# ziatdinovmax/GPim

Hardware: AMD Instinct MI355X
Metric: GP fit+predict grid-points/sec (higher is better)
Workload: dtype f64; 1 GPU; C2: 256x256 synthetic twisted-lattice image, 25% observed (N=16384, M=65536, d=2), Matern52 exact GP, T=100 Adam its (lr 0.1) + predict; one image per GPU; N=16384, M=65536, kernel=Matern52

## Files before the change

### gpim_amd/_lib.py

```python
import contextlib
import ctypes
import os

import torch

_HERE = os.path.dirname(os.path.abspath(__file__))
LIB_PATH = os.path.join(_HERE, "libgpimhip.so")

OK, E_BADARG, E_HIP, E_NOT_PD, E_NOMEM = 0, -1, -2, -3, -4
KERNEL_IDS = {"RBF": 0, "Matern52": 1, "RationalQuadratic": 2}
ACQ_IDS = {"cb": 0, "ei": 1, "poi": 2}
MAX_DIM, MAX_PARAMS = 4, 8

c_dp = ctypes.c_void_p


class ModelStruct(ctypes.Structure):
    _fields_ = [("kernel", ctypes.c_int32), ("dim", ctypes.c_int32), ("n_ls", ctypes.c_int32),
                ("reserved", ctypes.c_int32), ("amp_lo", ctypes.c_double), ("amp_hi", ctypes.c_double),
                ("ls_lo", ctypes.c_double * MAX_DIM), ("ls_hi", ctypes.c_double * MAX_DIM),
                ("jitter", ctypes.c_double)]


class VgpStruct(ctypes.Structure):
# ... 109 lines not shown
    "gpimhip_nll_grad_batched": (ctypes.c_int, [ctypes.c_void_p, ctypes.POINTER(ModelStruct), c_dp, ctypes.c_int64, c_dp,
                                                ctypes.c_int64, ctypes.c_int32, c_dp, c_dp, c_dp]),
    "gpimhip_acquire_exact": (ctypes.c_int, [ctypes.c_void_p, ctypes.POINTER(ModelStruct), c_dp, c_dp, ctypes.c_int64,
                                             c_dp, c_dp, ctypes.c_int64, c_dp, ctypes.c_int64, ctypes.c_int32,
                                             ctypes.c_double, ctypes.c_double, c_dp, c_dp, c_dp, c_dp]),
    "gpimhip_thin_batch": (ctypes.c_int, [ctypes.c_void_p, c_dp, c_dp, ctypes.c_int32, ctypes.c_int32, c_dp,
                                          ctypes.c_double, ctypes.c_int32, c_dp, c_dp]),
    "gpimhip_dist_vec_forward": (ctypes.c_int, [ctypes.c_void_p, c_dp, ctypes.c_int64, ctypes.c_int32, ctypes.c_int32,
                                                c_dp, c_dp, c_dp, c_dp]),
    "gpimhip_dist_vec_backward": (ctypes.c_int, [ctypes.c_void_p, c_dp, ctypes.c_int64, ctypes.c_int32, ctypes.c_int32,
                                                 c_dp, c_dp, c_dp, c_dp]),
    "gpimhip_matvec_t": (ctypes.c_int, [ctypes.c_void_p, c_dp, ctypes.c_int64, ctypes.c_int64, ctypes.c_int64, c_dp,
                                        c_dp]),
    "gpimhip_step_plan_host": (ctypes.c_int, [ctypes.c_int32, ctypes.c_int32, ctypes.POINTER(ctypes.c_int32),
                                              ctypes.c_int64, ctypes.POINTER(ctypes.c_int64)]),
    "gpimhip_step_plan_host_f32": (ctypes.c_int, [ctypes.c_int32, ctypes.c_int32, ctypes.POINTER(ctypes.c_int32),
                                                  ctypes.c_int64, ctypes.POINTER(ctypes.c_int64),
                                                  ctypes.POINTER(ctypes.c_int32)]),
    "gpimhip_vgp_nll_grad": (ctypes.c_int, [ctypes.c_void_p, ctypes.POINTER(ModelStruct), ctypes.POINTER(VgpStruct), c_dp,
                                            c_dp, ctypes.c_int64, c_dp, c_dp, c_dp]),
    "gpimhip_fit_vgp": (ctypes.c_int, [ctypes.c_void_p, ctypes.POINTER(ModelStruct), ctypes.POINTER(VgpStruct), c_dp, c_dp,
                                       ctypes.c_int64, c_dp, ctypes.c_double, ctypes.c_int32, c_dp, c_dp]),
    "gpimhip_predict_vgp": (ctypes.c_int, [ctypes.c_void_p, ctypes.POINTER(ModelStruct), ctypes.POINTER(VgpStruct), c_dp,
                                           c_dp, ctypes.c_int64, c_dp, c_dp, ctypes.c_int64, c_dp, c_dp]),
    "gpimhip_sm_kmat": (ctypes.c_int, [ctypes.c_void_p, ctypes.POINTER(SmStruct), c_dp, ctypes.c_int64, c_dp, ctypes.c_int64,
                                       c_dp, c_dp, ctypes.c_int64]),
    "gpimhip_sm_nll_grad": (ctypes.c_int, [ctypes.c_void_p, ctypes.POINTER(SmStruct), c_dp, c_dp, ctypes.c_int64, c_dp, c_dp,
                                           c_dp]),
    "gpimhip_fit_sm": (ctypes.c_int, [ctypes.c_void_p, ctypes.POINTER(SmStruct), c_dp, c_dp, ctypes.c_int64, c_dp,
                                      ctypes.c_double, ctypes.c_int32, c_dp, c_dp]),
# ... 124 lines not shown
```

### gpim_amd/csrc/api.hip

```cpp
#include <math.h>
#include <stdio.h>
#include <string.h>
#include <stdlib.h>
#include <algorithm>
#include <chrono>
#include <atomic>
#include <mutex>
#include "common.hpp"
#include "border.hpp"
#include "vgp.hpp"
#include "sm.hpp"
#include "sample.hpp"

static thread_local std::string g_err;
void gpim_set_error(const std::string& s) { g_err = s; }

static int deal_chunk(int ntiles = 1 << 30) { return std::max(1, std::min(64, ntiles / 512)); }
#define EAGER_MIN_PANELS 12
#define OUTER_W 4

template <typename T>
static int dev_alloc(gpimhip_ctx* h, T** p, int64_t count) {
    void* q = nullptr;
    hipError_t e = hipMalloc(&q, (size_t)count * sizeof(T));
    if (e != hipSuccess) {
        gpim_set_error(std::string("hipMalloc failed: ") + hipGetErrorString(e));
        return GPIMHIP_E_NOMEM;
    }
    *p = (T*)q;
    h->bytes += count * (int64_t)sizeof(T);
    return GPIMHIP_OK;
}
template <typename T>
static void dev_free(gpimhip_ctx* h, T** p, int64_t count) {
// ... 67 lines not shown
    }
    HIP_TRY(hipMemsetAsync(h->fin_counter, 0, (size_t)B * sizeof(uint32_t), h->stream));
    if (matrices) {
        HIP_TRY(hipMemsetAsync(h->Tm, 0, (size_t)mat_doubles(h, B * np * ld) * sizeof(double), h->stream));
        HIP_TRY(hipMemsetAsync(h->B, 0, (size_t)mat_doubles(h, B * np * ld) * sizeof(double), h->stream));
    }
    if (h->fp32 && h->refine_cap < 10 * (int64_t)B * np) {
        dev_free(h, &h->refine, h->refine_cap);
        h->refine_cap = 0;
        if ((rc = dev_alloc(h, &h->refine, 10 * (int64_t)B * np))) {
            ws_release_matrix(h);
            return rc;
        }
        h->refine_cap = 10 * (int64_t)B * np;
    }
    if (matrices) {
        rc = plan_ensure(h, (int)nb);
        if (rc == GPIMHIP_OK) rc = h->fp32 ? step_plan_ensure(h, (int)nb) : step_plan_ensure_inv(h, (int)nb);
        if (rc != GPIMHIP_OK) { ws_release_matrix(h); return rc; }
    }
    return GPIMHIP_OK;
}
int ws_ensure(gpimhip_ctx* h, int64_t N) { return ws_ensure_b(h, N, h->nbatch, 0); }
static int ws_ensure_padded(gpimhip_ctx* h, int64_t N) { return ws_ensure_b(h, N, h->nbatch, 1); }

static void ws_release_predict(gpimhip_ctx* h) {
    dev_free(h, &h->Ks, mat_doubles(h, h->ks_batch * h->ks_rows * (h->ks_cols + 16)));
    dev_free(h, &h->colpart, h->ks_batch * (h->ks_rows / NB) * h->ks_cols);
    dev_free(h, &h->mean_tmp, h->ks_batch * h->ks_cols);
    for (auto& pl : h->pred_lists) dev_free(h, &pl.tiles, pl.n);
// ... 127 lines not shown
    HIP_TRY(hipStreamSynchronize(h->stream));
    P.nb = nb;
    return GPIMHIP_OK;
}

static GemmArgs gemm_args(const double* A, int64_t lda, const double* B, int64_t ldb, double* C, int64_t ldc,
                          double alpha, double beta, const TileDesc* tiles, int n, int64_t rows) {
    GemmArgs g;
    memset(&g, 0, sizeof(g));
    g.A = A; g.lda = lda; g.B = B; g.ldb = ldb; g.C = C; g.ldc = ldc;
    g.alpha = alpha; g.beta = beta; g.tiles = tiles; g.ntiles = n;
    g.sA = rows * lda; g.sB = rows * ldb; g.sC = rows * ldc;
    return g;
}

struct SideStreams {
    hipStream_t capture = nullptr;
    bool capture_tried = false;
};
static std::mutex g_side_mutex;
static SideStreams g_side[64];
static std::atomic<int> g_side_generation{0};
static void side_refresh(gpimhip_ctx* h) {
    const int g = g_side_generation.load();
    if (h->side_generation == g) return;
    h->side_generation = g;
    h->capture_stream = nullptr;
    h->capture_stream_tried = false;
}
static std::mutex g_capture_mutex[64];
// ... 9 lines not shown
        if (!S.capture_tried) {
            S.capture_tried = true;
            if (hipStreamCreateWithFlags(&S.capture, hipStreamNonBlocking) != hipSuccess) S.capture = nullptr;
        }
        h->capture_stream = S.capture;
    }
    return h->capture_stream;
}

int launch_potrf(gpimhip_ctx* h, double* A, int64_t np, int64_t ld, int32_t* info) {
    return launch_potrf_steps(h, A, np, ld, info, nullptr);
}

int launch_trtri(gpimhip_ctx* h, double* A, double* Tm, int64_t np, int64_t ld) {
    const int nb = (int)(np / NB);
    GP_TRY(plan_ensure(h, nb));
    const LinalgPlan& P = h->plan;
    GP_TRY(launch_diag_inv_copy(h, A, ld, nb));
    for (size_t lv = 0; lv < P.tri_t.size(); ++lv) {
        GemmArgs g1 = gemm_args(A, ld, A, ld, Tm, ld, 1.0, 0.0, P.d_tiles + P.tri_t[lv].off, P.tri_t[lv].n, h->np);
        g1.chunk = deal_chunk(g1.ntiles);
        g1.krev = 1;
        GP_TRY(launch_gemm(h, false, true, EPI_STORE, g1));
        GemmArgs g2 = gemm_args(A, ld, Tm, ld, A, ld, -1.0, 0.0, P.d_tiles + P.tri_x[lv].off, P.tri_x[lv].n, h->np);
        g2.chunk = deal_chunk(g2.ntiles);
        GP_TRY(launch_gemm(h, false, true, EPI_STORE, g2));
    }
    return GPIMHIP_OK;
}

int launch_potrf_inv(gpimhip_ctx* h, double* A, double* Tm, int64_t np, int64_t ld, int32_t* info, int rag) {
    if (!h->fp32) return launch_potrf_steps(h, A, np, ld, info, Tm, rag);
    { StageTimer t(h, 0); GP_TRY(launch_potrf_steps(h, A, np, ld, info, nullptr)); }
    StageTimer t(h, 1);
    return launch_trtri(h, A, Tm, np, ld);
}

int launch_lauum(gpimhip_ctx* h, const double* A, double* B, int64_t np, int64_t ld, int rag) {
    const int nb = (int)(np / NB);
    GP_TRY(plan_ensure(h, nb));
    const LinalgPlan& P = h->plan;
    GemmArgs g = gemm_args(A, ld, A, ld, B, ld, 1.0, 0.0, P.d_tiles + P.lauum.off, P.lauum.n, h->np);
    g.chunk = deal_chunk(g.ntiles);
    g.krev = 1;
    g.rag = h->fp32 ? 0 : rag;
    return launch_gemm(h, true, true, EPI_STORE, g);
}

static BorderWs* bws(const gpimhip_ctx* h) { return (BorderWs*)h->border; }
static bool border_on(const gpimhip_ctx* h) { return h->refl.mask && h->border && bws(h)->M > 0; }

static void border_free_bufs(gpimhip_ctx* h, BorderWs* w) {
    dev_free(h, &w->C, (int64_t)w->B * w->np * w->mp);
    dev_free(h, &w->Y, (int64_t)w->B * w->np * w->mp);
// ... 133 lines not shown
        GP_TRY(launch_kmat(h, m, X, N, nullptr, N, h->theta, 0.0, 1, h->A, ld, np, np, 1, 1, x_bs, x_bs, np * ld));
    GP_TRY(launch_potrf_inv(h, h->A, h->Tm, np, ld, h->info, rag_of(N, np)));
    return solve_vectors(h, m, X, x_bs, N, defer_alpha);
}

struct IterTable : FinalizeIter { bool theta_carried; };

static int loss_grad_at_u(gpimhip_ctx* h, const gpimhip_model_t* m, const double* X, int64_t x_bs, int64_t N,
                          double* u, int do_adam, AdamStep st, double* loss_out, double* grad_out,
                          double* hist_row, const IterTable* tab = nullptr) {
    const int64_t np = h->np;
    const bool modern = !h->refl.mask && !getenv("GPIMHIP_NO_FUSED_FINALIZE");
    const bool fused = modern && np <= 8192;
    const bool carried = modern && tab && tab->theta_carried;
    const bool defer = fused && alpha_deferrable(h);
    GP_TRY(factor_at_u(h, m, X, x_bs, N, u, carried, defer));
    { StageTimer t(h, 2); GP_TRY(launch_lauum(h, h->A, h->B, np, h->ld, rag_of(N, np))); }
    if (h->refl.mask) {
        const bool bd = border_on(h);
        if (bd) GP_TRY(border_iter(h, N, true));
        const double* bscal = bd ? bws(h)->scal : nullptr;
        GP_TRY(launch_grad_reduce_refl(h, m, h->B, h->ld, X, N, (int)(np / NB), h->alpha, x_bs));
        if (tab)
            return launch_finalize_coupled(h, m, N, np, u, do_adam, st, nullptr, nullptr, nullptr, tab->iter, tab->bc, tab->T,
                                           tab->hist_base, tab->loss_base, bscal);
        return launch_finalize_coupled(h, m, N, np, u, do_adam, st, loss_out, grad_out, hist_row, nullptr, nullptr, 0, nullptr,
                                       nullptr, bscal);
    }
    if (fused) {
        const double* ap = defer ? h->gemv_part : nullptr;
// ... 161 lines not shown
int gpimhip_destroy(gpimhip_handle h) {
    if (!h) return GPIMHIP_OK;
    (void)hipSetDevice(h->device);
    (void)hipStreamSynchronize(h->stream);
    vfe_release(h);
    kron_release(h);
    vgp_release(h);
    sm_release(h);
    border_release(h);
    sample_release(h);
    ws_release_matrix(h);
    ws_release_predict(h);
    dev_free(h, &h->keys, h->keys_cap);
    if (h->sel_scratch) dev_free(h, &h->sel_scratch, (int64_t)sel_scratch_bytes());
    dev_free(h, &h->acq_tmp, h->acq_tmp_cap);
    dev_free(h, &h->refine, h->refine_cap);
    dev_free(h, &h->bc, h->bc_cap);
    dev_free(h, &h->theta1, 1);
    dev_free(h, &h->info, 4);
    if (h->plan.d_tiles) (void)hipFree(h->plan.d_tiles);
    step_plan_release(h);
    dist_plan_release(h);
    for (auto e : h->ra_ev)
        if (e) (void)hipEventDestroy(e);
    if (h->pinned_info) (void)hipHostFree(h->pinned_info);
    delete h;
    return GPIMHIP_OK;
}

int64_t gpimhip_workspace_bytes(gpimhip_handle h) {
// ... 53 lines not shown
                             (size_t)Mv * sizeof(double), (size_t)N, hipMemcpyDeviceToDevice, h->stream));
    return GPIMHIP_OK;
}

int gpimhip_potrf(gpimhip_handle h, double* A, int64_t n, int64_t ld, int32_t* info) {
    FP64_ONLY(h);
    if (!h || !A || n < 1 || ld < n || !info) return GPIMHIP_E_BADARG;
    HIP_TRY(hipSetDevice(h->device));
    h->nbatch = 1;
    GP_TRY(ws_ensure(h, n));
    const int64_t np = h->np;
    HIP_TRY(hipMemsetAsync(info, 0, sizeof(int32_t), h->stream));
    GP_TRY(launch_pad_matrix_in(h, A, n, ld, h->A, np));
    GP_TRY(launch_potrf(h, h->A, np, np, info));
    GP_TRY(launch_pad_matrix_out_lower(h, h->A, np, A, n, ld));
    return GPIMHIP_OK;
}

static int fit_impl(gpimhip_ctx* h, const gpimhip_model_t* m, const double* X, int64_t x_bs, const double* y,
                    int64_t N, int B, double* u, double lr, int32_t T, double* hist_out, double* loss_out) {
    HIP_TRY(hipSetDevice(h->device));
    h->nbatch = B;
    HIP_TRY(hipMemsetAsync(h->info, 0, sizeof(int32_t), h->stream));
    HIP_TRY(hipMemsetAsync(h->info + 1, 0x7f, sizeof(int32_t), h->stream));
    h->fit_completed = T;
    if (T == 0) return GPIMHIP_OK;
    GP_TRY(upload_bc_table(h, lr, T));
    if (use_small_path(N) && !h->refl.mask) {
        GP_TRY(launch_fit_small(h, m, X, x_bs, y, (int)N, u, h->bc, h->bc + T, T, hist_out, loss_out, nullptr));
        return finish_and_check(h);
// ... 8 lines not shown
    const bool carry = !h->refl.mask && !getenv("GPIMHIP_NO_FUSED_FINALIZE");
    if (carry) GP_TRY(launch_theta(h, m, u));
    const IterTable tab{{h->iter, h->bc, T, hist_out, loss_out}, carry};
    const AdamStep st = adam_step_init();
    return run_fit_iterations(h, T, FIT_LOOP_DENSE,
                              [&] { return loss_grad_at_u(h, m, X, x_bs, N, u, 1, st, nullptr, nullptr, nullptr, &tab); });
}


struct VgpGroup { int T, nrep; const VgpDev* st; };

static int predict_cols(gpimhip_ctx* h, const gpimhip_model_t* m, const double* X, int64_t x_bs, int64_t N, int B,
                        const double* Xs, int64_t M, double* mean_out, double* var_out, const VgpGroup* vgrp = nullptr) {
    const int64_t np = h->np;
    const int nb = (int)(np / NB);
    if (!h->fp32 && fused_predict_fits(np) && !h->refl.mask)
        return launch_predict_fused(h, m, X, x_bs, N, Xs, M, mean_out, var_out, nullptr, nullptr, -1, 0.0, nullptr, 0.0,
                                    nullptr);
    int64_t mc = pad_to(M, NB);
    const int64_t cap = std::max<int64_t>(NB, ((int64_t)1 << 27) / np / B / NB * NB);
    mc = std::min(mc, cap);
    GP_TRY(ws_ensure_predict(h, np, mc));
    const int64_t mcap = h->ks_cols, kld = mcap + 16;
    const bool bd = border_on(h);
    if (bd) GP_TRY(border_ensure_r(h, mcap));
    for (int64_t m0 = 0; m0 < M; m0 += mc) {
        const int64_t cnt = std::min(mc, M - m0);
        const int64_t cpad = pad_to(cnt, NB);
        if (h->refl.mask)
            GP_TRY(launch_kmat_refl(h, m, X, N, Xs + m0 * m->dim, cnt, h->theta, h->Ks, kld, np, cpad, 0, x_bs, 0, np * kld,
// ... 43 lines not shown
        else GP_TRY(launch_predict_var(h, mcap, nb, m0, cnt, var_out, M));
    }
    return GPIMHIP_OK;
}

static int predict_impl(gpimhip_ctx* h, const gpimhip_model_t* m, const double* X, int64_t x_bs, const double* y,
                        int64_t N, int B, const double* u, const double* Xs, int64_t M, double* mean_out,
                        double* var_out) {
    HIP_TRY(hipSetDevice(h->device));
    h->nbatch = B;
    GP_TRY(ws_ensure_padded(h, N));
    const int64_t np = h->np;
    HIP_TRY(hipMemsetAsync(h->info, 0, sizeof(int32_t), h->stream));
    GP_TRY(launch_pad_copy(h, y, N, h->ypad, np));
    if (border_on(h)) GP_TRY(border_ensure(h));
    GP_TRY(factor_at_u(h, m, X, x_bs, N, u));
    if (border_on(h)) {
        GP_TRY(launch_lauum(h, h->A, h->B, np, h->ld, rag_of(N, np)));
        GP_TRY(border_iter(h, N, false));
    }
    GP_TRY(predict_cols(h, m, X, x_bs, N, B, Xs, M, mean_out, var_out));
    return finish_and_check(h);
}

int gpimhip_nll_grad(gpimhip_handle h, const gpimhip_model_t* m, const double* X, const double* y, int64_t N,
                     const double* u, double* loss_out, double* grad_out) {
    if (!h || !X || !y || !u || N < 1) return GPIMHIP_E_BADARG;
    GP_TRY(check_model(m));
    HIP_TRY(hipSetDevice(h->device));
    h->nbatch = 1;
// ... 1166 lines not shown
```

### gpim_amd/csrc/cholstep.hip

```cpp
#include <stdlib.h>
#include <string.h>
#include <algorithm>
#include <functional>
#include "potf2_body.hpp"
#include "gemm_body.hpp"

#ifndef STEP_W
#define STEP_W 4
#endif

#define TILE_COPY (1 << 19)

struct StepArgs {
    double* A; int64_t ld; int kblk; int nb;
    double* dinv_all; double* dinvB_all; double* logdet; int32_t* info;
    int col_off;
    int potf2;
    int pb_off, pb_cnt, hb_off, hb_cnt, swap;
    double* Tm;
    double* Pcopy;
    GemmArgs g;
};

template <int FTM, int FTN, bool ALONE, bool RAG = false>
__global__ __launch_bounds__(NTH, ALONE ? 2 : 4) void chol_step_kernel(StepArgs a) {
    constexpr int SM0 = POTF2_SMEM_DOUBLES > gemm_smem_doubles<FTM, FTN, 2>() ? POTF2_SMEM_DOUBLES : gemm_smem_doubles<FTM, FTN, 2>();
    static_assert(SM0 * 8 <= 80 * 1024, "two workgroups per CU");
    constexpr int SM = ALONE ? 84 * 128 : SM0;
    __shared__ __attribute__((aligned(16))) double smem[SM];
    const int b = a.swap ? blockIdx.y : blockIdx.x;
    const int by = a.swap ? blockIdx.x : blockIdx.y;
    if (b >= 8) {
        if (by >= a.hb_cnt) return;
        const int pb = by + a.hb_off;
        int quad;
        const int pos = gemm_tile_pos<FTM, FTN>(a.g.ntiles, a.g.chunk, b - 8, quad);
        TileDesc t = a.g.tiles[pos];
        const int kind = (t.kb1 >> 16) & 7;
        const bool copy = (t.kb1 & TILE_COPY) != 0;
        t.kb1 &= 0xffff;
        if (kind == 0) {
            if (copy && a.Pcopy) {
                GemmArgs g = a.g;
                g.C2 = a.Pcopy + (int64_t)pb * (NB * NB);
                gemm_tile_core<false, false, EPI_STORE, 8, FTM, FTN, 2, RAG>(g, t, quad, pb, smem);
            } else {
                gemm_tile_core<false, false, EPI_STORE, 8, FTM, FTN, 2, RAG>(a.g, t, quad, pb, smem);
            }
        } else {
            GemmArgs g = a.g;
            if (kind <= 2) { g.C = a.Tm; g.alpha = 1.0; g.beta = kind == 2 ? 1.0 : 0.0; }
// ... 628 lines not shown
static int launch_step(gpimhip_ctx* h, StepArgs& a, bool potf2, int n, int q, const int* split = nullptr, bool two_per_cu = false) {
    const int B = h->nbatch;
    a.potf2 = potf2 ? 1 : 0;
    if (!potf2 && n == 0) return GPIMHIP_OK;
    a.pb_off = a.hb_off = 0; a.pb_cnt = a.hb_cnt = B; a.swap = 0;
    dim3 grid(n ? 8 + q * n : 1, B);
    bool alone = potf2;
    if (q == 4 && two_per_cu) alone = false;
    if (split) {
        a.pb_off = split[0]; a.pb_cnt = potf2 ? split[1] : 0; a.hb_off = split[2]; a.hb_cnt = n ? split[3] : 0; a.swap = 1;
        grid = dim3(std::max(a.pb_cnt, a.hb_cnt), n ? 8 + q * n : 1);
        alone = false;
        if (grid.x == 0) return GPIMHIP_OK;
        if (grid.y > 65535) { gpim_set_error("step launch: tile list too long for a split batch"); return GPIMHIP_E_BADARG; }
    }
    if (a.g.rag && n) {
        if (q == 4 && alone) hipLaunchKernelGGL((chol_step_kernel<64, 64, true, true>), grid, dim3(NTH), 0, h->stream, a);
        else if (q == 4) hipLaunchKernelGGL((chol_step_kernel<64, 64, false, true>), grid, dim3(NTH), 0, h->stream, a);
        else if (q == 2) hipLaunchKernelGGL((chol_step_kernel<128, 64, false, true>), grid, dim3(NTH), 0, h->stream, a);
        else hipLaunchKernelGGL((chol_step_kernel<128, 128, false, true>), grid, dim3(NTH), 0, h->stream, a);
    } else if (q == 4 && alone) hipLaunchKernelGGL((chol_step_kernel<64, 64, true>), grid, dim3(NTH), 0, h->stream, a);
    else if (q == 4) hipLaunchKernelGGL((chol_step_kernel<64, 64, false>), grid, dim3(NTH), 0, h->stream, a);
    else if (q == 2) hipLaunchKernelGGL((chol_step_kernel<128, 64, false>), grid, dim3(NTH), 0, h->stream, a);
    else hipLaunchKernelGGL((chol_step_kernel<128, 128, false>), grid, dim3(NTH), 0, h->stream, a);
    HIP_TRY(hipGetLastError());
    return GPIMHIP_OK;
}

static int launch_solve_diag(gpimhip_ctx* h, double* A, int64_t ld, int j, int nb, int ndiag, int b_off, int cnt,
                             bool fused = false) {
    if (j + 1 >= nb || cnt <= 0) return GPIMHIP_OK;
    if (fused && cnt <= 4) {
        const int below = nb - j - 2;
        if ((36 + 4 * below) * cnt <= 256)
            hipLaunchKernelGGL(panel_solve_diag_kernel<16>, dim3(36 + 4 * below, cnt), dim3(512), 0, h->stream, A, ld, j, nb,
                               (const double*)h->dinvB, (const double*)h->pcopy, b_off);
        else
            hipLaunchKernelGGL(panel_solve_diag_kernel<32>, dim3(10 + 2 * below, cnt), dim3(512), 0, h->stream, A, ld, j, nb,
                               (const double*)h->dinvB, (const double*)h->pcopy, b_off);
// ... 4 lines not shown
        hipLaunchKernelGGL(panel_solve_kernel<4>, dim3(4 * (nb - j - 1), cnt), dim3(256), 0, h->stream, A, ld, j, nb,
                           (const double*)h->dinvB, b_off);
    else
        hipLaunchKernelGGL(panel_solve_kernel<2>, dim3(4 * (nb - j - 1), cnt), dim3(256), 0, h->stream, A, ld, j, nb,
                           (const double*)h->dinvB, b_off);
    HIP_TRY(hipGetLastError());
    if (ndiag > 0) {
        hipLaunchKernelGGL(diag_update_kernel, dim3(10 * ndiag, cnt), dim3(256), 0, h->stream, A, ld, j, nb, b_off);
        HIP_TRY(hipGetLastError());
    }
    return GPIMHIP_OK;
}

int launch_potrf_steps(gpimhip_ctx* h, double* A, int64_t np, int64_t ld, int32_t* info, double* Tm, int rag) {
    if (h->fp32) return launch_potrf_steps_f32(h, A, np, ld, info);
    const int nb = (int)(np / NB);
    if (Tm) GP_TRY(step_plan_ensure_inv(h, nb));
    else GP_TRY(step_plan_ensure(h, nb));
    const StepPlan& P = Tm ? h->splan_inv : h->splan;
    const int B = h->nbatch;
    const int host_max_batch = 4;
    StepArgs a;
    a.A = A; a.ld = ld; a.nb = nb; a.Tm = Tm;
    a.dinv_all = h->dinv; a.dinvB_all = h->dinvB; a.logdet = h->logdet_part; a.info = info;
    a.col_off = 0;
    a.Pcopy = h->pcopy;
    const bool no_fused = getenv("GPIMHIP_NO_FUSED_FD") != nullptr;
    auto fused = [&](int j) { return !no_fused && h->pcopy && P.copy[j] && P.diag[j].n == 1 && !(rag && j + 2 == nb); };
    {
        StageTimer t(h, 0);
// ... 37 lines not shown
        a.kblk = -1;
        for (const PlanRange& r : P.post) {
            a.g = nt_update(A, ld, P.d_tiles + r.off, r.n, h->np);
            a.g.chunk = std::max(1, std::min(64, r.n / 512));
            a.g.rag = rag;
            const int64_t nt = (int64_t)r.n * B;
            GP_TRY(launch_step(h, a, false, r.n, nt <= 320 ? 4 : (nt <= 1000 ? 2 : 1)));
        }
    }
    return GPIMHIP_OK;
}

int launch_panel_chain(gpimhip_ctx* h, double* A, int64_t ld, int p0, int p1, int nb, const TileDesc* tiles,
                       const PlanRange* colfill, int32_t* info) {
    const int B = h->nbatch;
    StepArgs a;
    a.A = A; a.ld = ld; a.nb = nb; a.Tm = nullptr;
    a.dinv_all = h->dinv; a.dinvB_all = h->dinvB; a.logdet = h->logdet_part; a.info = info;
    a.col_off = 0;
    a.Pcopy = nullptr;
    for (int j = p0; j < p1; ++j) {
        a.kblk = j;
        const PlanRange f = colfill[j - p0];
        a.g = nt_update(A, ld, tiles + f.off, f.n, h->np);
        a.g.chunk = 1;
        GP_TRY(launch_step(h, a, true, f.n, f.n <= 128 ? 4 : 2));
        GP_TRY(launch_solve_diag(h, A, ld, j, nb, std::max(0, p1 - j - 1), 0, B));
    }
    return GPIMHIP_OK;
}
// ... 1 lines not shown
```

### gpim_amd/csrc/common.hpp

```cpp
#pragma once
#include <hip/hip_runtime.h>
#include <stdint.h>
#include <functional>
#include <string>
#include <vector>
#include <utility>
#include "../../include/gpimhip.h"

#define NB 128
#define GEMM_BK 16
#define MAXP GPIMHIP_MAX_PARAMS

void gpim_set_error(const std::string& s);

#define HIP_TRY(expr)                                                              \
    do {                                                                           \
        hipError_t _e = (expr);                                                    \
        if (_e != hipSuccess) {                                                    \
            gpim_set_error(std::string(#expr) + ": " + hipGetErrorString(_e));     \
            return GPIMHIP_E_HIP;                                                  \
        }                                                                          \
    } while (0)

#define GP_TRY(expr)                      \
// ... 134 lines not shown
    unsigned long long* keys = nullptr;
    int64_t keys_cap = 0;
    double* acq_tmp = nullptr; int64_t acq_tmp_cap = 0;
    char* sel_scratch = nullptr;
    int fit_completed = 0;
    int32_t* pinned_info = nullptr;
    hipEvent_t ra_ev[2] = {nullptr, nullptr};
    void* vfe = nullptr;
    void* kron = nullptr;
    void* vgp = nullptr;
    void* sm = nullptr;
    void* border = nullptr;
    void* sample = nullptr;
    double* refine = nullptr; int64_t refine_cap = 0;
    int fp32 = 0;
};

#define FP64_ONLY(h)                                                                                      \
    do {                                                                                                  \
        if ((h) && (h)->fp32) {                                                                           \
            gpim_set_error("this entry point needs a double-precision handle (gpimhip_set_precision(h, 64))"); \
            return GPIMHIP_E_BADARG;                                                                      \
        }                                                                                                 \
    } while (0)

static inline int64_t pad_to(int64_t n, int64_t m) { return (n + m - 1) / m * m; }
static inline int rag_of(int64_t N, int64_t np) {
    const int64_t last = N - (np - NB);
    return (np >= 2 * NB && last > 0 && last <= 64) ? (int)(np / NB) : 0;
}
// ... 121 lines not shown
    double alpha, beta;
    const TileDesc* tiles; int ntiles;
    int cj_max;
    int cmap;
    int chunk;
    int inplace;
    int rag;
    int krev;
    int kfix0, kfix1;
    int rect_rows, rect_cols;
    double* colpart; int64_t ld_colpart;
    double* C2;
    int shape_div;
    int64_t sA, sB, sC, sColpart;
    int bshift;
};
int launch_gemm(gpimhip_ctx* h, bool a_km, bool b_km, int epi, const GemmArgs& g);
int launch_gemm_f32(gpimhip_ctx* h, bool a_km, bool b_km, int epi, const GemmArgs& g);
```

### gpim_amd/csrc/gemm.hip

```cpp
#include <stdlib.h>
#include "gemm_body.hpp"

template <bool A_KM, bool B_KM, int EPI, int NW, int TSM, int TSN>
__global__ __launch_bounds__(NW * 64, 2) void gemm_tiles_kernel(GemmArgs g) {
    __shared__ __attribute__((aligned(16))) double smem[gemm_smem_doubles<TSM, TSN>()];
    gemm_tile_body<A_KM, B_KM, EPI, NW, TSM, TSN>(g, (int)blockIdx.x, (int)blockIdx.y, smem);
}

static int mid_tiles() {
    static const int v = 1100;
    return v;
}

template <bool A_KM, bool B_KM, int EPI>
static int launch_one(gpimhip_ctx* h, const GemmArgs& g) {
    if (g.ntiles <= 0) return GPIMHIP_OK;
    const int64_t total = (int64_t)g.ntiles * h->nbatch / (g.shape_div > 1 ? g.shape_div : 1);
    const int tile64_max = 640;
    const bool small = total <= tile64_max;
    if (EPI == EPI_STORE && small && !g.inplace)
        hipLaunchKernelGGL((gemm_tiles_kernel<A_KM, B_KM, EPI_STORE, 4, 64, 64>), dim3(g.ntiles * 4, h->nbatch),
                           dim3(256), 0, h->stream, g);
    else if (EPI == EPI_STORE && small)
        hipLaunchKernelGGL((gemm_tiles_kernel<A_KM, B_KM, EPI_STORE, 8, 64, 128>), dim3(g.ntiles * 2, h->nbatch),
                           dim3(512), 0, h->stream, g);
    else if (EPI == EPI_STORE && total > 256 && total <= mid_tiles())
        hipLaunchKernelGGL((gemm_tiles_kernel<A_KM, B_KM, EPI, 8, 128, 128>), dim3(g.ntiles, h->nbatch), dim3(512),
                           24 * 1024, h->stream, g);
    else if (total <= 256 || (!A_KM && !B_KM))
        hipLaunchKernelGGL((gemm_tiles_kernel<A_KM, B_KM, EPI, 8, 128, 128>), dim3(g.ntiles, h->nbatch), dim3(512), 0,
                           h->stream, g);
    else
        hipLaunchKernelGGL((gemm_tiles_kernel<A_KM, B_KM, EPI, 4, 128, 128>), dim3(g.ntiles, h->nbatch), dim3(256), 0,
                           h->stream, g);
    HIP_TRY(hipGetLastError());
    return GPIMHIP_OK;
}

static int launch_gemm_f64(gpimhip_ctx* h, bool a_km, bool b_km, int epi, const GemmArgs& g) {
    if (epi == EPI_STORE) {
        if (!a_km && !b_km) return launch_one<false, false, EPI_STORE>(h, g);
        if (!a_km && b_km) return launch_one<false, true, EPI_STORE>(h, g);
        if (a_km && b_km) return launch_one<true, true, EPI_STORE>(h, g);
    } else {
        if (!a_km && b_km) return launch_one<false, true, EPI_COLSUMSQ>(h, g);
    }
    gpim_set_error("launch_gemm: unsupported operand layout combination");
    return GPIMHIP_E_BADARG;
}

int launch_gemm(gpimhip_ctx* h, bool a_km, bool b_km, int epi, const GemmArgs& g) {
    return h->fp32 ? launch_gemm_f32(h, a_km, b_km, epi, g) : launch_gemm_f64(h, a_km, b_km, epi, g);
}
```

### gpim_amd/csrc/gemm_body.hpp

```cpp
#pragma once
#include "common.hpp"

typedef double d4 __attribute__((ext_vector_type(4)));
typedef double d2 __attribute__((ext_vector_type(2)));

#define LD_MK (GEMM_BK + 2)
#ifndef MK_GROUP
#define MK_GROUP 130
#endif

template <bool KM, int NT, int TS>
__device__ __forceinline__ void stage_load(d2 (&r)[8 * TS / NT], const double* __restrict__ base, int64_t ld,
                                           int64_t mrow0, int64_t kcol0, int tid) {
#pragma unroll
    for (int i = 0; i < 8 * TS / NT; ++i) {
        const int c = tid + NT * i;
        if (!KM) {
            const int row = c >> 3, c16 = c & 7;
            r[i] = *reinterpret_cast<const d2*>(base + (mrow0 + row) * ld + kcol0 + c16 * 2);
        } else {
            const int krow = c / (TS / 2), c16 = c % (TS / 2);
            r[i] = *reinterpret_cast<const d2*>(base + (kcol0 + krow) * ld + mrow0 + c16 * 2);
        }
    }
// ... 72 lines not shown
    if (!KM) return lds[(m0 + (lane & 15)) * LD_MK + kk * 4 + (lane >> 4)];
    return lds[(kk * 4 + (lane >> 4)) * (TS + 16) + m0 + (lane & 15)];
}

template <int TSM, int TSN, int NSTG = 2>
__host__ __device__ constexpr int gemm_smem_doubles() {
    constexpr int TSX = TSM > TSN ? TSM : TSN;
    return 2 * NSTG * ((TSX * LD_MK > GEMM_BK * (TSX + 16)) ? TSX * LD_MK : GEMM_BK * (TSX + 16));
}
template <int TSM, int TSN>
__device__ __forceinline__ int gemm_tile_pos(int n, int chunk, int bx, int& quad) {
    constexpr int QUADS = (128 / TSM) * (128 / TSN);
    const int b = bx / QUADS;
    quad = bx % QUADS;
    if (QUADS > 1) return b;
    if (chunk == 0) {
        const int q = n >> 3, r = n & 7, x = b & 7, yy = b >> 3;
        return (x < r ? x * (q + 1) : r * (q + 1) + (x - r) * q) + yy;
    }
    const int C = chunk, full = (n / (8 * C)) * (8 * C);
    if (b < full) {
        const int x = b & 7, y = b >> 3, round = y / C;
        return (round * 8 + ((round & 1) ? 7 - x : x)) * C + (y % C);
    }
    return b;
}

template <bool A_KM, bool B_KM, int EPI, int NW, int TSM, int TSN, int NSTG = 2, bool RAG = false>
__device__ __forceinline__ void gemm_tile_core(GemmArgs g, TileDesc t, const int quad, const int by, double* __restrict__ smem);

template <bool A_KM, bool B_KM, int EPI, int NW, int TSM, int TSN, int NSTG = 2>
__device__ __forceinline__ void gemm_tile_body(GemmArgs g, const int bx, const int by, double* __restrict__ smem) {
    int quad;
    const int p = gemm_tile_pos<TSM, TSN>(g.ntiles, g.chunk, bx, quad);
    TileDesc t;
    if (g.rect_cols > 0) {
        const int per = 8 * g.rect_cols, s = p / per, q = p - s * per, rows_here = min(8, g.rect_rows - 8 * s);
        t.ci = 8 * s + q % rows_here;
        t.cj = q / rows_here;
        t.kb0 = g.kfix0;
        t.kb1 = g.kfix1;
    } else {
        t = g.tiles[p];
    }
    if (g.rag) gemm_tile_core<A_KM, B_KM, EPI, NW, TSM, TSN, NSTG, true>(g, t, quad, by, smem);
    else gemm_tile_core<A_KM, B_KM, EPI, NW, TSM, TSN, NSTG, false>(g, t, quad, by, smem);
}

template <bool A_KM, bool B_KM, int EPI, int NW, int TSM, int TSN, int NSTG, bool RAG>
// ... 238 lines not shown
```

### include/gpimhip.h

```cpp
#ifndef GPIMHIP_H
#define GPIMHIP_H

#include <stdint.h>

#ifdef __cplusplus
extern "C" {
#endif

#define GPIMHIP_OK            0
#define GPIMHIP_E_BADARG     -1
#define GPIMHIP_E_HIP        -2
#define GPIMHIP_E_NOT_PD     -3
#define GPIMHIP_E_NOMEM      -4

#define GPIMHIP_KERNEL_RBF       0
#define GPIMHIP_KERNEL_MATERN52  1
#define GPIMHIP_KERNEL_RQ        2

#define GPIMHIP_ACQ_CB   0
#define GPIMHIP_ACQ_EI   1
#define GPIMHIP_ACQ_POI  2

#define GPIMHIP_MAX_DIM  4
#define GPIMHIP_MAX_PARAMS 8
// ... 181 lines not shown

int gpimhip_set_reflection_shard(gpimhip_handle h, int32_t pb_off, int32_t pb_stride, int32_t nblocks_total, int32_t raw);

int gpimhip_set_border(gpimhip_handle h, int32_t M, const int32_t* q, const double* coef);
int gpimhip_nll_grad_batched(gpimhip_handle h, const gpimhip_model_t* m, const double* X, int64_t x_stride, const double* y,
                             int64_t N, int32_t B, const double* u, double* loss_out, double* grad_out);
int gpimhip_refl_sums(gpimhip_handle h, const gpimhip_model_t* m, const double* X, const double* y, int64_t N, int32_t B,
                      const double* u, double* sums_out);

int gpimhip_thin_batch(gpimhip_handle h, const double* vals, const int64_t* flat_idx, int32_t n, int32_t d,
                       const int64_t* shape, double dscale, int32_t max_out, int32_t* keep_out,
                       int32_t* nkeep_out);

int gpimhip_step_plan_host(int32_t nb, int32_t with_inverse, int32_t* out, int64_t cap, int64_t* n_out);

int gpimhip_step_plan_host_f32(int32_t nb, int32_t with_inverse, int32_t* out, int64_t cap, int64_t* n_out,
                               int32_t* diag_out);

int gpimhip_timing_enable(gpimhip_handle h, int enable);
int gpimhip_timing_read(gpimhip_handle h, int stage, double* total_ms, int64_t* count);

int gpimhip_fit_completed(gpimhip_handle h);

int gpimhip_shutdown(void);

int gpimhip_sync(gpimhip_handle h);

#ifdef __cplusplus
}
#endif
// ... 2 lines not shown
```

Measured before the change: 8831 grid-points/s.

## Add atomic ticket-based dynamic tile scheduling for GEMM and Cholesky step kernels

Workgroups beyond the number that fit resident on the device now claim their tile index from a global atomic counter instead of taking it from the static blockIdx mapping. The first wave keeps the static swizzled order. The aim is to balance load across CUs when tile costs vary, for example in triangular trailing updates. Ticket counters live in a per-context buffer that is memset at scope entry, which adds memsets, atomics, extra LDS syncs and occupancy queries per launch. The change also adds host helpers to dump the workspace matrix and the tile map.

Result: no change. 8862 grid-points/s (median of 6 runs) (+0.3%).

```diff
diff --git a/gpim_amd/_lib.py b/gpim_amd/_lib.py
--- a/gpim_amd/_lib.py
+++ b/gpim_amd/_lib.py
@@ -147,6 +147,9 @@
                                         c_dp]),
     "gpimhip_step_plan_host": (ctypes.c_int, [ctypes.c_int32, ctypes.c_int32, ctypes.POINTER(ctypes.c_int32),
                                               ctypes.c_int64, ctypes.POINTER(ctypes.c_int64)]),
+    "gpimhip_workspace_matrix": (ctypes.c_int, [ctypes.c_void_p, ctypes.c_int32, ctypes.c_int64, c_dp, ctypes.c_int64]),
+    "gpimhip_tile_map_host": (ctypes.c_int, [ctypes.c_int32, ctypes.c_int32, ctypes.c_int32,
+                                             ctypes.POINTER(ctypes.c_int32)]),
     "gpimhip_step_plan_host_f32": (ctypes.c_int, [ctypes.c_int32, ctypes.c_int32, ctypes.POINTER(ctypes.c_int32),
                                                   ctypes.c_int64, ctypes.POINTER(ctypes.c_int64),
                                                   ctypes.POINTER(ctypes.c_int32)]),
diff --git a/gpim_amd/csrc/api.hip b/gpim_amd/csrc/api.hip
--- a/gpim_amd/csrc/api.hip
+++ b/gpim_amd/csrc/api.hip
@@ -18,6 +18,11 @@
 static int deal_chunk(int ntiles = 1 << 30) { return std::max(1, std::min(64, ntiles / 512)); }
 #define EAGER_MIN_PANELS 12
 #define OUTER_W 4
+
+static bool tickets_enabled() {
+    const char* v = getenv("GPIMHIP_TILE_TICKETS");
+    return !(v && atoi(v) == 0);
+}
 
 template <typename T>
 static int dev_alloc(gpimhip_ctx* h, T** p, int64_t count) {
@@ -115,6 +120,7 @@
         }
         h->refine_cap = 10 * (int64_t)B * np;
     }
+    if (tickets_enabled()) GP_TRY(dev_grow(h, &h->ticket, &h->ticket_cap, std::max<int64_t>(1024, (4 * nb + 64) * (int64_t)B)));
     if (matrices) {
         rc = plan_ensure(h, (int)nb);
         if (rc == GPIMHIP_OK) rc = h->fp32 ? step_plan_ensure(h, (int)nb) : step_plan_ensure_inv(h, (int)nb);
@@ -272,6 +278,38 @@
     return g;
 }
 
+int resident_workgroups(gpimhip_ctx* h, const void* kernel, int threads, size_t dyn_lds, int* cache) {
+    if (*cache > 0) return *cache;
+    int per_cu = 0, cus = 0;
+    if (hipOccupancyMaxActiveBlocksPerMultiprocessor(&per_cu, kernel, threads, dyn_lds) != hipSuccess || per_cu < 1 ||
+        hipDeviceGetAttribute(&cus, hipDeviceAttributeMultiprocessorCount, h->device) != hipSuccess || cus < 1) {
+        (void)hipGetLastError();
+        return 1 << 30;
+    }
+    return *cache = per_cu * cus;
+}
+
+int ticket_assign(gpimhip_ctx* h, GemmArgs& g, int resident, int quads) {
+    g.ticket = nullptr;
+    g.n_static = 0;
+    if (h->ticket_depth == 0 || !h->ticket || g.ntiles <= 0 || !tickets_enabled()) return GPIMHIP_OK;
+    const char* forced = getenv("GPIMHIP_TICKET_STATIC");
+    const int64_t want = forced ? atoll(forced) : std::max(0, resident) / quads;
+    const int n_static = tile_static_count(g.ntiles, g.chunk, want);
+    if (n_static >= g.ntiles) return GPIMHIP_OK;
+    const int B = h->nbatch;
+    if (B > h->ticket_cap) return GPIMHIP_OK;
+    if (h->ticket_dirty || h->ticket_next + B > h->ticket_cap) {
+        HIP_TRY(hipMemsetAsync(h->ticket, 0, (size_t)h->ticket_cap * sizeof(uint32_t), h->stream));
+        h->ticket_dirty = false;
+        h->ticket_next = 0;
+    }
+    g.ticket = h->ticket + h->ticket_next;
+    g.n_static = n_static;
+    h->ticket_next += B;
+    return GPIMHIP_OK;
+}
+
 struct SideStreams {
     hipStream_t capture = nullptr;
     bool capture_tried = false;
@@ -311,6 +349,7 @@
 
 int launch_trtri(gpimhip_ctx* h, double* A, double* Tm, int64_t np, int64_t ld) {
     const int nb = (int)(np / NB);
+    TicketScope tickets(h);
     GP_TRY(plan_ensure(h, nb));
     const LinalgPlan& P = h->plan;
     GP_TRY(launch_diag_inv_copy(h, A, ld, nb));
@@ -335,6 +374,7 @@
 
 int launch_lauum(gpimhip_ctx* h, const double* A, double* B, int64_t np, int64_t ld, int rag) {
     const int nb = (int)(np / NB);
+    TicketScope tickets(h);
     GP_TRY(plan_ensure(h, nb));
     const LinalgPlan& P = h->plan;
     GemmArgs g = gemm_args(A, ld, A, ld, B, ld, 1.0, 0.0, P.d_tiles + P.lauum.off, P.lauum.n, h->np);
@@ -498,6 +538,7 @@
     const bool fused = modern && np <= 8192;
     const bool carried = modern && tab && tab->theta_carried;
     const bool defer = fused && alpha_deferrable(h);
+    TicketScope tickets(h);
     GP_TRY(factor_at_u(h, m, X, x_bs, N, u, carried, defer));
     { StageTimer t(h, 2); GP_TRY(launch_lauum(h, h->A, h->B, np, h->ld, rag_of(N, np))); }
     if (h->refl.mask) {
@@ -689,6 +730,8 @@
     dev_free(h, &h->keys, h->keys_cap);
     if (h->sel_scratch) dev_free(h, &h->sel_scratch, (int64_t)sel_scratch_bytes());
     dev_free(h, &h->acq_tmp, h->acq_tmp_cap);
+    dev_free(h, &h->ticket, h->ticket_cap);
+    h->ticket_cap = 0;
     dev_free(h, &h->refine, h->refine_cap);
     dev_free(h, &h->bc, h->bc_cap);
     dev_free(h, &h->theta1, 1);
@@ -772,6 +815,15 @@
     GP_TRY(launch_pad_matrix_in(h, A, n, ld, h->A, np));
     GP_TRY(launch_potrf(h, h->A, np, np, info));
     GP_TRY(launch_pad_matrix_out_lower(h, h->A, np, A, n, ld));
+    return GPIMHIP_OK;
+}
+
+int gpimhip_workspace_matrix(gpimhip_handle h, int32_t which, int64_t n, double* out, int64_t ld) {
+    if (!h || !out || n < 1 || n > h->np || ld < n || which < 0 || which > 1 || !h->A || !h->B) return GPIMHIP_E_BADARG;
+    FP64_ONLY(h);
+    HIP_TRY(hipSetDevice(h->device));
+    GP_TRY(launch_pad_matrix_out_lower(h, which == 0 ? h->A : h->B, h->ld, out, n, ld));
+    HIP_TRY(hipStreamSynchronize(h->stream));
     return GPIMHIP_OK;
 }
 
@@ -810,6 +862,7 @@
                         const double* Xs, int64_t M, double* mean_out, double* var_out, const VgpGroup* vgrp = nullptr) {
     const int64_t np = h->np;
     const int nb = (int)(np / NB);
+    TicketScope tickets(h);
     if (!h->fp32 && fused_predict_fits(np) && !h->refl.mask)
         return launch_predict_fused(h, m, X, x_bs, N, Xs, M, mean_out, var_out, nullptr, nullptr, -1, 0.0, nullptr, 0.0,
                                     nullptr);
@@ -883,6 +936,7 @@
     HIP_TRY(hipMemsetAsync(h->info, 0, sizeof(int32_t), h->stream));
     GP_TRY(launch_pad_copy(h, y, N, h->ypad, np));
     if (border_on(h)) GP_TRY(border_ensure(h));
+    TicketScope tickets(h);
     GP_TRY(factor_at_u(h, m, X, x_bs, N, u));
     if (border_on(h)) {
         GP_TRY(launch_lauum(h, h->A, h->B, np, h->ld, rag_of(N, np)));
diff --git a/gpim_amd/csrc/cholstep.hip b/gpim_amd/csrc/cholstep.hip
--- a/gpim_amd/csrc/cholstep.hip
+++ b/gpim_amd/csrc/cholstep.hip
@@ -33,8 +33,8 @@
     if (b >= 8) {
         if (by >= a.hb_cnt) return;
         const int pb = by + a.hb_off;
-        int quad;
-        const int pos = gemm_tile_pos<FTM, FTN>(a.g.ntiles, a.g.chunk, b - 8, quad);
+        int quad, pos;
+        if (!gemm_tile_claim<FTM, FTN>(a.g, b - 8, by, smem, pos, quad)) return;
         TileDesc t = a.g.tiles[pos];
         const int kind = (t.kb1 >> 16) & 7;
         const bool copy = (t.kb1 & TILE_COPY) != 0;
@@ -693,15 +693,16 @@
         if (grid.x == 0) return GPIMHIP_OK;
         if (grid.y > 65535) { gpim_set_error("step launch: tile list too long for a split batch"); return GPIMHIP_E_BADARG; }
     }
-    if (a.g.rag && n) {
-        if (q == 4 && alone) hipLaunchKernelGGL((chol_step_kernel<64, 64, true, true>), grid, dim3(NTH), 0, h->stream, a);
-        else if (q == 4) hipLaunchKernelGGL((chol_step_kernel<64, 64, false, true>), grid, dim3(NTH), 0, h->stream, a);
-        else if (q == 2) hipLaunchKernelGGL((chol_step_kernel<128, 64, false, true>), grid, dim3(NTH), 0, h->stream, a);
-        else hipLaunchKernelGGL((chol_step_kernel<128, 128, false, true>), grid, dim3(NTH), 0, h->stream, a);
-    } else if (q == 4 && alone) hipLaunchKernelGGL((chol_step_kernel<64, 64, true>), grid, dim3(NTH), 0, h->stream, a);
-    else if (q == 4) hipLaunchKernelGGL((chol_step_kernel<64, 64, false>), grid, dim3(NTH), 0, h->stream, a);
-    else if (q == 2) hipLaunchKernelGGL((chol_step_kernel<128, 64, false>), grid, dim3(NTH), 0, h->stream, a);
-    else hipLaunchKernelGGL((chol_step_kernel<128, 128, false>), grid, dim3(NTH), 0, h->stream, a);
+    const bool rag = a.g.rag && n;
+    const int k = (q == 4 ? (alone ? 0 : 1) : (q == 2 ? 2 : 3)) + (rag ? 4 : 0);
+    void (*const kernels[8])(StepArgs) = {
+        chol_step_kernel<64, 64, true>, chol_step_kernel<64, 64, false>, chol_step_kernel<128, 64, false>, chol_step_kernel<128, 128, false>,
+        chol_step_kernel<64, 64, true, true>, chol_step_kernel<64, 64, false, true>, chol_step_kernel<128, 64, false, true>,
+        chol_step_kernel<128, 128, false, true>};
+    static int resident[8] = {0, 0, 0, 0, 0, 0, 0, 0};
+    a.g.ticket = nullptr;
+    if (n && !potf2) GP_TRY(ticket_assign(h, a.g, resident_workgroups(h, (const void*)kernels[k], NTH, 0, &resident[k]) - 8, q));
+    hipLaunchKernelGGL(kernels[k], grid, dim3(NTH), 0, h->stream, a);
     HIP_TRY(hipGetLastError());
     return GPIMHIP_OK;
 }
@@ -736,6 +737,7 @@
 
 int launch_potrf_steps(gpimhip_ctx* h, double* A, int64_t np, int64_t ld, int32_t* info, double* Tm, int rag) {
     if (h->fp32) return launch_potrf_steps_f32(h, A, np, ld, info);
+    TicketScope tickets(h);
     const int nb = (int)(np / NB);
     if (Tm) GP_TRY(step_plan_ensure_inv(h, nb));
     else GP_TRY(step_plan_ensure(h, nb));
@@ -803,6 +805,7 @@
 int launch_panel_chain(gpimhip_ctx* h, double* A, int64_t ld, int p0, int p1, int nb, const TileDesc* tiles,
                        const PlanRange* colfill, int32_t* info) {
     const int B = h->nbatch;
+    TicketScope tickets(h);
     StepArgs a;
     a.A = A; a.ld = ld; a.nb = nb; a.Tm = nullptr;
     a.dinv_all = h->dinv; a.dinvB_all = h->dinvB; a.logdet = h->logdet_part; a.info = info;
diff --git a/gpim_amd/csrc/common.hpp b/gpim_amd/csrc/common.hpp
--- a/gpim_amd/csrc/common.hpp
+++ b/gpim_amd/csrc/common.hpp
@@ -172,6 +172,10 @@
     void* sample = nullptr;
     double* refine = nullptr; int64_t refine_cap = 0;
     int fp32 = 0;
+    uint32_t* ticket = nullptr;
+    int64_t ticket_cap = 0, ticket_next = 0;
+    int ticket_depth = 0;
+    bool ticket_dirty = true;
 };
 
 #define FP64_ONLY(h)                                                                                      \
@@ -323,6 +327,47 @@
     int shape_div;
     int64_t sA, sB, sC, sColpart;
     int bshift;
-};
+    uint32_t* ticket;
+    int n_static;
+};
+
+__host__ __device__ static inline int tile_pos_static(int n, int chunk, int b) {
+    if (chunk == 0) {
+        const int q = n >> 3, r = n & 7, x = b & 7, yy = b >> 3;
+        return (x < r ? x * (q + 1) : r * (q + 1) + (x - r) * q) + yy;
+    }
+    const int C = chunk, full = (n / (8 * C)) * (8 * C);
+    if (b < full) {
+        const int x = b & 7, y = b >> 3, round = y / C;
+        return (round * 8 + ((round & 1) ? 7 - x : x)) * C + (y % C);
+    }
+    return b;
+}
+static inline int tile_static_count(int ntiles, int chunk, int64_t want) {
+    if (want >= ntiles) return ntiles;
+    if (want <= 0) return 0;
+    const int unit = 8 * (chunk > 0 ? chunk : 1);
+    return (int)(want / unit * unit);
+}
+__host__ __device__ static inline int tile_pos_ticket(int n, int chunk, int n_static, int t) {
+    if (chunk != 0) return n_static + t;
+    const int q = n >> 3, r = n & 7, s = n_static >> 3, l1 = q + 1 - s, l0 = q - s;
+    if (t < r * l1) return (t / l1) * (q + 1) + s + t % l1;
+    t -= r * l1;
+    if (l0 <= 0) return n;
+    return r * (q + 1) + (t / l0) * q + s + t % l0;
+}
+
 int launch_gemm(gpimhip_ctx* h, bool a_km, bool b_km, int epi, const GemmArgs& g);
+struct TicketScope {
+    gpimhip_ctx* h;
+    explicit TicketScope(gpimhip_ctx* h_) : h(h_) {
+        if (h->ticket_depth++ == 0) { h->ticket_next = 0; h->ticket_dirty = true; }
+    }
+    ~TicketScope() { --h->ticket_depth; }
+    TicketScope(const TicketScope&) = delete;
+    TicketScope& operator=(const TicketScope&) = delete;
+};
+int ticket_assign(gpimhip_ctx* h, GemmArgs& g, int resident, int quads);
+int resident_workgroups(gpimhip_ctx* h, const void* kernel, int threads, size_t dyn_lds, int* cache);
 int launch_gemm_f32(gpimhip_ctx* h, bool a_km, bool b_km, int epi, const GemmArgs& g);
diff --git a/gpim_amd/csrc/gemm.hip b/gpim_amd/csrc/gemm.hip
--- a/gpim_amd/csrc/gemm.hip
+++ b/gpim_amd/csrc/gemm.hip
@@ -12,29 +12,30 @@
     return v;
 }
 
+template <int QUADS>
+static int launch_shape(gpimhip_ctx* h, void (*kernel)(GemmArgs), int threads, size_t dyn_lds, int* resident, GemmArgs g) {
+    GP_TRY(ticket_assign(h, g, resident_workgroups(h, (const void*)kernel, threads, dyn_lds, resident), QUADS));
+    hipLaunchKernelGGL(kernel, dim3(g.ntiles * QUADS, h->nbatch), dim3(threads), dyn_lds, h->stream, g);
+    HIP_TRY(hipGetLastError());
+    return GPIMHIP_OK;
+}
+
 template <bool A_KM, bool B_KM, int EPI>
 static int launch_one(gpimhip_ctx* h, const GemmArgs& g) {
     if (g.ntiles <= 0) return GPIMHIP_OK;
+    static int resident[5] = {0, 0, 0, 0, 0};
     const int64_t total = (int64_t)g.ntiles * h->nbatch / (g.shape_div > 1 ? g.shape_div : 1);
     const int tile64_max = 640;
     const bool small = total <= tile64_max;
     if (EPI == EPI_STORE && small && !g.inplace)
-        hipLaunchKernelGGL((gemm_tiles_kernel<A_KM, B_KM, EPI_STORE, 4, 64, 64>), dim3(g.ntiles * 4, h->nbatch),
-                           dim3(256), 0, h->stream, g);
-    else if (EPI == EPI_STORE && small)
-        hipLaunchKernelGGL((gemm_tiles_kernel<A_KM, B_KM, EPI_STORE, 8, 64, 128>), dim3(g.ntiles * 2, h->nbatch),
-                           dim3(512), 0, h->stream, g);
-    else if (EPI == EPI_STORE && total > 256 && total <= mid_tiles())
-        hipLaunchKernelGGL((gemm_tiles_kernel<A_KM, B_KM, EPI, 8, 128, 128>), dim3(g.ntiles, h->nbatch), dim3(512),
-                           24 * 1024, h->stream, g);
-    else if (total <= 256 || (!A_KM && !B_KM))
-        hipLaunchKernelGGL((gemm_tiles_kernel<A_KM, B_KM, EPI, 8, 128, 128>), dim3(g.ntiles, h->nbatch), dim3(512), 0,
-                           h->stream, g);
-    else
-        hipLaunchKernelGGL((gemm_tiles_kernel<A_KM, B_KM, EPI, 4, 128, 128>), dim3(g.ntiles, h->nbatch), dim3(256), 0,
-                           h->stream, g);
-    HIP_TRY(hipGetLastError());
-    return GPIMHIP_OK;
+        return launch_shape<4>(h, gemm_tiles_kernel<A_KM, B_KM, EPI_STORE, 4, 64, 64>, 256, 0, &resident[0], g);
+    if (EPI == EPI_STORE && small)
+        return launch_shape<2>(h, gemm_tiles_kernel<A_KM, B_KM, EPI_STORE, 8, 64, 128>, 512, 0, &resident[1], g);
+    if (EPI == EPI_STORE && total > 256 && total <= mid_tiles())
+        return launch_shape<1>(h, gemm_tiles_kernel<A_KM, B_KM, EPI, 8, 128, 128>, 512, 24 * 1024, &resident[2], g);
+    if (total <= 256 || (!A_KM && !B_KM))
+        return launch_shape<1>(h, gemm_tiles_kernel<A_KM, B_KM, EPI, 8, 128, 128>, 512, 0, &resident[3], g);
+    return launch_shape<1>(h, gemm_tiles_kernel<A_KM, B_KM, EPI, 4, 128, 128>, 256, 0, &resident[4], g);
 }
 
 static int launch_gemm_f64(gpimhip_ctx* h, bool a_km, bool b_km, int epi, const GemmArgs& g) {
@@ -49,6 +50,14 @@
     return GPIMHIP_E_BADARG;
 }
 
+extern "C" int gpimhip_tile_map_host(int32_t ntiles, int32_t chunk, int32_t n_static, int32_t* out) {
+    if (ntiles < 1 || chunk < 0 || n_static < 0 || !out) return GPIMHIP_E_BADARG;
+    const int ns = tile_static_count(ntiles, chunk, n_static);
+    for (int b = 0; b < ns; ++b) out[b] = tile_pos_static(ntiles, chunk, b);
+    for (int t = 0; t < ntiles - ns; ++t) out[ns + t] = tile_pos_ticket(ntiles, chunk, ns, t);
+    return ns;
+}
+
 int launch_gemm(gpimhip_ctx* h, bool a_km, bool b_km, int epi, const GemmArgs& g) {
     return h->fp32 ? launch_gemm_f32(h, a_km, b_km, epi, g) : launch_gemm_f64(h, a_km, b_km, epi, g);
 }
diff --git a/gpim_amd/csrc/gemm_body.hpp b/gpim_amd/csrc/gemm_body.hpp
--- a/gpim_amd/csrc/gemm_body.hpp
+++ b/gpim_amd/csrc/gemm_body.hpp
@@ -110,16 +110,23 @@
     const int b = bx / QUADS;
     quad = bx % QUADS;
     if (QUADS > 1) return b;
-    if (chunk == 0) {
-        const int q = n >> 3, r = n & 7, x = b & 7, yy = b >> 3;
-        return (x < r ? x * (q + 1) : r * (q + 1) + (x - r) * q) + yy;
-    }
-    const int C = chunk, full = (n / (8 * C)) * (8 * C);
-    if (b < full) {
-        const int x = b & 7, y = b >> 3, round = y / C;
-        return (round * 8 + ((round & 1) ? 7 - x : x)) * C + (y % C);
-    }
-    return b;
+    return tile_pos_static(n, chunk, b);
+}
+template <int TSM, int TSN>
+__device__ __forceinline__ bool gemm_tile_claim(const GemmArgs& g, int bx, int slot, double* smem, int& p, int& quad) {
+    constexpr int QUADS = (128 / TSM) * (128 / TSN);
+    if (g.ticket == nullptr || bx / QUADS < g.n_static) {
+        p = gemm_tile_pos<TSM, TSN>(g.ntiles, g.chunk, bx, quad);
+        return true;
+    }
+    uint32_t* box = reinterpret_cast<uint32_t*>(smem);
+    if (threadIdx.x == 0) *box = __hip_atomic_fetch_add(g.ticket + slot, 1u, __ATOMIC_RELAXED, __HIP_MEMORY_SCOPE_AGENT);
+    __syncthreads();
+    const int t = __builtin_amdgcn_readfirstlane((int)*box);
+    __syncthreads();
+    quad = t % QUADS;
+    p = QUADS > 1 ? g.n_static + t / QUADS : tile_pos_ticket(g.ntiles, g.chunk, g.n_static, t);
+    return p < g.ntiles;
 }
 
 template <bool A_KM, bool B_KM, int EPI, int NW, int TSM, int TSN, int NSTG = 2, bool RAG = false>
@@ -127,8 +134,8 @@
 
 template <bool A_KM, bool B_KM, int EPI, int NW, int TSM, int TSN, int NSTG = 2>
 __device__ __forceinline__ void gemm_tile_body(GemmArgs g, const int bx, const int by, double* __restrict__ smem) {
-    int quad;
-    const int p = gemm_tile_pos<TSM, TSN>(g.ntiles, g.chunk, bx, quad);
+    int quad, p;
+    if (!gemm_tile_claim<TSM, TSN>(g, bx, by, smem, p, quad)) return;
     TileDesc t;
     if (g.rect_cols > 0) {
         const int per = 8 * g.rect_cols, s = p / per, q = p - s * per, rows_here = min(8, g.rect_rows - 8 * s);
diff --git a/include/gpimhip.h b/include/gpimhip.h
--- a/include/gpimhip.h
+++ b/include/gpimhip.h
@@ -219,6 +219,10 @@
 
 int gpimhip_step_plan_host(int32_t nb, int32_t with_inverse, int32_t* out, int64_t cap, int64_t* n_out);
 
+int gpimhip_workspace_matrix(gpimhip_handle h, int32_t which, int64_t n, double* out, int64_t ld);
+
+int gpimhip_tile_map_host(int32_t ntiles, int32_t chunk, int32_t n_static, int32_t* out);
+
 int gpimhip_step_plan_host_f32(int32_t nb, int32_t with_inverse, int32_t* out, int64_t cap, int64_t* n_out,
                                int32_t* diag_out);
 
```
